# SiftScience/kafka-assigner

Measured on NVIDIA H100. Metric: partition-replica assignments/sec, higher is better.
Workload: dtype int32

## Files before the change

### kafka_assigner_b200/csrc/kassign.cu

```cuda
#include "kassign_stage.cuh"
#include "kassign_order.cuh"
#include "kassign_json.cuh"
#include "kassign_score.cuh"
#include "kassign_waves.cuh"
#include "kassign_waves_json.cuh"

#include <algorithm>
#include <climits>
#include <cmath>
#include <cstdio>
#include <cstdlib>
#include <cstring>
#include <map>
#include <new>
#include <string>
#include <unordered_map>
#include <vector>

#include "../../include/kassign.h"

namespace {

constexpr int KA_SM_COUNT_FALLBACK = 132;
constexpr size_t KA_SMEM_BUDGET = 200 * 1024;
// ... 162 lines not shown

template <typename F>
void for_each_event(ka_ctx* c, F f) {
    const struct { cudaEvent_t* e; size_t n; bool timed; } pools[] = {
        {c->ev, sizeof(c->ev) / sizeof(cudaEvent_t), true},
        {&c->ev_pipe[0][0], sizeof(c->ev_pipe) / sizeof(cudaEvent_t), true},
        {&c->ev_chain[0][0], sizeof(c->ev_chain) / sizeof(cudaEvent_t), true},
        {&c->ev_in, 1, false},
        {c->ev_stage, KA_MAX_BLOCKS, false},
        {&c->ev_chain_in, 1, false},
        {c->ev_b1, KA_MAX_CHAIN_EVENTS, false},
        {c->ev_b2, KA_MAX_CHAIN_EVENTS, false},
        {&c->ev_emit_done, 1, false},
        {c->ev_json_in, KA_MAX_JSON_FRAGS, false},
        {c->ev_json_scan, KA_MAX_JSON_FRAGS, false},
        {&c->ev_out_done, 1, false},
    };
    for (const auto& p : pools)
        for (size_t i = 0; i < p.n; ++i) f(p.e[i], p.timed);
}

int park_counters(ka_ctx* c) {
    if (c->br.N == 0 || !c->d_ctr8.p) return KA_OK;
    std::vector<int32_t> h((size_t)c->br.N * KA_MAX_SLOTS);
    KA_CUDA(cudaMemcpy(h.data(), c->d_ctr8.p, h.size() * 4, cudaMemcpyDeviceToHost));
    for (int i = 0; i < c->br.N; ++i) {
        const int32_t* row = h.data() + (size_t)i * KA_MAX_SLOTS;
        bool nz = false;
        for (int r = 0; r < KA_MAX_SLOTS; ++r) nz |= row[r] != 0;
        if (nz) c->parked[c->broker_id[i]] = std::vector<int32_t>(row, row + KA_MAX_SLOTS);
        else c->parked.erase(c->broker_id[i]);
    }
    return KA_OK;
}

int check_brokers(int N, const int32_t* broker_id, const int32_t* broker_rack) {
    if (N < 0 || (N > 0 && (!broker_id || !broker_rack))) return KA_ERR_BAD_ARG;
    if (N > 65535) return KA_ERR_LIMIT;
    for (int i = 0; i < N; ++i) {
        if (i > 0 && broker_id[i] <= broker_id[i - 1]) return KA_ERR_BAD_ARG;
        if (broker_rack[i] < 0 || broker_rack[i] >= 65535) return KA_ERR_BAD_ARG;
    }
    return KA_OK;
}

struct BrokerTable {
    int lut_mode = KA_LUT_SMEM, min_id = 0, lut_off = 0;
    uint32_t range = 0;
    std::vector<uint16_t> blob, glut;
    int blob_bytes() const { return (int)(blob.size() * 2); }
    KaBrokers device(int N, const uint16_t* d_blob, const uint16_t* d_glut, const int32_t* d_broker_id) const {
        return KaBrokers{N, lut_mode, lut_off, blob_bytes(), min_id, range, d_blob, d_glut, d_broker_id};
    }
};

BrokerTable broker_table(int N, const int32_t* broker_id, const int32_t* broker_rack) {
    BrokerTable t;
    t.min_id = N > 0 ? broker_id[0] : 0;
    const uint64_t range64 = N > 0 ? (uint64_t)((int64_t)broker_id[N - 1] - (int64_t)broker_id[0]) + 1 : 0;
    const size_t npad = align16((size_t)std::max(N, 1) * 2) / 2;
    std::vector<uint16_t> rackc(std::max(N, 1), 0);
    {
        std::unordered_map<int32_t, int> seen;
        for (int i = 0; i < N; ++i) {
            auto it = seen.find(broker_rack[i]);
            if (it == seen.end()) it = seen.emplace(broker_rack[i], (int)seen.size()).first;
            rackc[i] = (uint16_t)it->second;
        }
    }
    size_t lut_elems = 0;
    if (range64 <= KA_LUT_SMEM_MAX_RANGE) {
        t.lut_mode = KA_LUT_SMEM;
        t.range = (uint32_t)range64;
        lut_elems = align16((size_t)std::max<uint64_t>(range64, 1) * 2) / 2;
    } else if (range64 <= KA_LUT_GLOBAL_MAX_RANGE) {
        t.lut_mode = KA_LUT_GLOBAL;
        t.range = (uint32_t)range64;
        t.glut.assign((size_t)range64, (uint16_t)KA_DEAD);
        for (int i = 0; i < N; ++i) t.glut[(size_t)((int64_t)broker_id[i] - t.min_id)] = (uint16_t)i;
    } else {
        t.lut_mode = KA_LUT_BSEARCH;
        t.range = 0;
    }
    t.lut_off = (int)npad;
    t.blob.assign(npad + lut_elems, (uint16_t)KA_DEAD);
    for (int i = 0; i < N; ++i) {
        t.blob[i] = rackc[i];
        if (t.lut_mode == KA_LUT_SMEM) t.blob[npad + (size_t)((int64_t)broker_id[i] - t.min_id)] = (uint16_t)i;
    }
    return t;
}

constexpr size_t KA_ORDER_SMEM_BUDGET = 226 * 1024;

int make_plan(int N, int blob_bytes, int64_t Q, int S, int Pmax, int64_t capmax, bool ragged, Plan& pl, ka_status* st) {
    if (Q >= (int64_t)1 << 31) return set_status(st, KA_ERR_LIMIT, -1, -1, INT_MAX, 0);
    pl.a_blob_bytes = blob_bytes;
    pl.a_load_kind = capmax <= 255 ? 0 : 1;
    const int lsz = pl.a_load_kind == 0 ? 1 : 2;
    pl.a_load_bytes = (int)align16((size_t)std::max(N, 1) * lsz);
    pl.a_slab_bytes = (int)align16((size_t)std::max(Pmax, 1) * S * 2);
    pl.a_cnt_bytes = (int)align16((size_t)std::max(Pmax, 1));
    pl.a_levels = (capmax > 1 || ragged) ? 1 : 0;
    if (pl.a_levels && Pmax > 32767) return set_status(st, KA_ERR_LIMIT, -1, -1, Pmax, N);
    pl.lv_owner_bytes = pl.a_levels ? (int)align16((size_t)std::max(N, 1) * 4) : 0;
    pl.lv_last_bytes = pl.a_levels ? (int)align16((size_t)std::max(N, 1) * 2) : 0;
    pl.lv_p_bytes = pl.a_levels ? (int)align16((size_t)(std::max(Pmax, 1) + 2) * 2) : 0;
    const size_t per_warp = (size_t)pl.a_load_bytes + pl.a_slab_bytes + pl.a_cnt_bytes + pl.lv_owner_bytes + pl.lv_last_bytes +
                            2 * (size_t)pl.lv_p_bytes;
    const size_t shared = 16 + (size_t)blob_bytes;
    if (shared + per_warp > KA_SMEM_BUDGET) return set_status(st, KA_ERR_LIMIT, -1, -1, Pmax, N);
    pl.a_warps = (int)std::min<size_t>(16, (KA_SMEM_BUDGET - shared) / per_warp);
    pl.a_smem = shared + per_warp * pl.a_warps;
    pl.rec_kind = S <= 3 ? 3 : (S == 4 ? 4 : 8);
    pl.rec_bytes = pl.rec_kind == 3 ? 16 : 32;
    const int cw = pl.rec_kind == 8 ? 8 : 4;
    const int max_nt = pl.rec_kind == 3 ? 1024 : (pl.rec_kind == 4 ? 512 : 256);
    const size_t ctr_bytes = pl.rec_kind == 3 ? (size_t)(std::max(N, 1) + 1) * 4 : (size_t)std::max(N, 1) * cw * 4;
    const int lg_max = pl.rec_kind == 3 ? 10 : 9, lg_min = 7;
    auto ring_bytes = [&](int l) { return ((size_t)KA_RING_STAGES << l) * pl.rec_bytes + 256; };
    int lg = lg_max;
    pl.b_gctr = 0;
    while (lg > lg_min && ctr_bytes + ring_bytes(lg) > KA_ORDER_SMEM_BUDGET) --lg;
    if (ctr_bytes + ring_bytes(lg) > KA_ORDER_SMEM_BUDGET) {
        pl.b_gctr = 1;
        lg = lg_max;
    }
    if (const char* e = std::getenv("KA_ORDER_GLOBAL_CTR")) pl.b_gctr = pl.b_gctr || std::atoi(e);
    pl.b_ring_log2 = lg;
    pl.b_smem = ring_bytes(lg) + (pl.b_gctr ? 0 : ctr_bytes);
    int64_t width = pl.a_levels ? std::min<int64_t>(Pmax, std::max<int64_t>(1, N / std::max(S, 1) / 2)) : Pmax;
    const int64_t cuts = (std::max<int64_t>(width, 1) + max_nt - 1) / max_nt;
    width = (std::max<int64_t>(width, 1) + cuts - 1) / cuts;
    int nt = (int)std::min<int64_t>(max_nt, ((width + 31) / 32) * 32);
    if (const char* e = std::getenv("KA_ORDER_THREADS")) nt = std::atoi(e);
    nt = std::max(32, std::min(max_nt, (nt / 32) * 32));
    nt = std::min(nt, (KA_RING_STAGES - 1) << lg);
    pl.b_threads = nt;
    return KA_OK;
}

template <typename K>
cudaError_t allow_smem(K kernel, size_t bytes) {
    return cudaFuncSetAttribute(kernel, cudaFuncAttributeMaxDynamicSharedMemorySize, (int)bytes);
}

struct Shape {
    int T = 0, P = 0, RF = 0, desired_rf = -1, S = 1;
    const int32_t* d_hash = nullptr;
    const int32_t* d_cur = nullptr;
    const int64_t* d_part_off = nullptr;
    const int64_t* d_rep_off = nullptr;
    int64_t Q = 0, R = 0;
    int Pmax = 0;
    int64_t capmax = 0;
};

int64_t dense_capmax(int P, int rf_t, int n) {
    return n > 0 && rf_t <= n ? ((int64_t)P * std::max(rf_t, 0) + n - 1) / n : 0;
}

Shape dense_shape(int T, int P, int RF, int desired_rf, int S, int N, const int32_t* d_hash = nullptr, const int32_t* d_cur = nullptr) {
    Shape sh{T, P, RF, desired_rf, S, d_hash, d_cur};
    sh.Q = (int64_t)T * P;
    sh.R = sh.Q * RF;
    sh.Pmax = P;
    sh.capmax = dense_capmax(P, desired_rf >= 0 ? desired_rf : RF, N);
    return sh;
}

Shape ragged_shape(int T, int64_t Q, int64_t R, int desired_rf, int S, int Pmax = 0, int64_t capmax = 0) {
    Shape sh{T, 0, 0, desired_rf, S};
    sh.Q = Q;
    sh.R = R;
    sh.Pmax = Pmax;
    sh.capmax = capmax;
    return sh;
}

int describe_block(const Shape& sh, int t0, int t1, int blk, int N, int blob_bytes, StageDesc& d, ka_status* st) {
    const bool ragged = sh.d_part_off != nullptr;
    d = StageDesc();
    d.topic_base = t0;
    d.T = t1 - t0;
    d.blk = blk;
    d.q0 = (int64_t)t0 * sh.P;
    d.Q = ragged ? sh.Q : (int64_t)d.T * sh.P;
    d.d_hash = sh.d_hash + t0;
    d.d_part_off = sh.d_part_off;
    d.d_rep_off = sh.d_rep_off;
    d.P = sh.P;
    d.RF = sh.RF;
    d.d_cur = sh.d_cur + d.q0 * sh.RF;
    d.desired_rf = sh.desired_rf;
    d.S = sh.S;
    d.Pmax = sh.Pmax;
    d.capmax = sh.capmax;
    return make_plan(N, blob_bytes, d.Q, d.S, d.Pmax, d.capmax, ragged, d.pl, st);
}

int reserve_scratch(ka_ctx* c, const StageDesc* ds, int K) {
    const StageDesc& e = ds[K - 1];
    const size_t q = (size_t)std::max<int64_t>(e.q0 + e.Q, 1);
    const size_t T = (size_t)std::max(e.topic_base + e.T, 1);
    KA_CUDA(c->run.reserve(q * ds[0].pl.rec_bytes + 256, q, T, T + K + 1, ds[0].pl.a_levels, 16));
    return KA_OK;
}

int reserve_io(ka_ctx* c, Shape& sh, bool ragged) {
    KA_CUDA(c->d_hash.reserve((size_t)std::max(sh.T, 1) * 4));
    if (ragged) {
        KA_CUDA(c->d_part_off.reserve((size_t)(sh.T + 1) * 8));
        KA_CUDA(c->d_rep_off.reserve((size_t)(sh.Q + 1) * 8));
    }
    KA_CUDA(c->d_cur.reserve((size_t)std::max<int64_t>(sh.R, 1) * 4));
    KA_CUDA(c->d_out.reserve((size_t)std::max<int64_t>(sh.Q, 1) * sh.S * 4));
    KA_CUDA(c->d_out_len.reserve((size_t)std::max<int64_t>(sh.Q, 1) * 4));
    sh.d_hash = c->d_hash.as<int32_t>();
    sh.d_cur = c->d_cur.as<int32_t>();
    if (ragged) {
        sh.d_part_off = c->d_part_off.as<int64_t>();
        sh.d_rep_off = c->d_rep_off.as<int64_t>();
    }
    return KA_OK;
}

int reset_flags(ka_ctx* c, cudaStream_t s) {
    c->h_pin->err_topic = -1;
    c->h_pin->spin_flag = -1;
    c->chain_used = 0;
    c->slot_timed[0] = c->slot_timed[1] = false;
    KA_CUDA(cudaMemsetAsync(c->run.flags.p, 0xFF, 2 * sizeof(int), s));
    return KA_OK;
}

template <typename LoadT, bool LEVELS, int SM, bool CAND>
cudaError_t launch_stage_t(ka_ctx* c, cudaStream_t s, const KaSolveParams& p, const Plan& pl, int T, int ncand, int* grid_x) {
    auto kern = ka_sticky_spread_kernel<LoadT, LEVELS, SM, CAND>;
    const int threads = pl.a_warps * 32;
    cudaError_t e = allow_smem(kern, pl.a_smem);
    if (e != cudaSuccess) return e;
    int occ = 1;
    e = cudaOccupancyMaxActiveBlocksPerMultiprocessor(&occ, kern, threads, pl.a_smem);
    if (e != cudaSuccess) return e;
    int grid = (T + pl.a_warps - 1) / pl.a_warps;
    grid = std::min(grid, std::max(1, std::max(1, occ) * c->sm_count / std::max(ncand, 1)));
    *grid_x = grid;
    kern<<<dim3(grid, std::max(ncand, 1)), threads, pl.a_smem, s>>>(p, pl.a_load_bytes, pl.a_slab_bytes, pl.a_cnt_bytes, pl.lv_owner_bytes,
                                                                 pl.lv_last_bytes, pl.lv_p_bytes);
    return cudaGetLastError();
}

template <typename LoadT, bool LEVELS, bool CAND>
cudaError_t launch_stage(ka_ctx* c, cudaStream_t s, const KaSolveParams& p, const Plan& pl, int T, int ncand, int* grid_x) {
    return p.S <= 3 ? launch_stage_t<LoadT, LEVELS, 3, CAND>(c, s, p, pl, T, ncand, grid_x)
                    : launch_stage_t<LoadT, LEVELS, 8, CAND>(c, s, p, pl, T, ncand, grid_x);
}

void reset_plans(ka_ctx* c) {
    for (int32_t& v : c->order_plan) v = 0;
    for (int32_t& v : c->stage_plan) v = 0;
}

template <bool CAND>
int launch_stage_plan(ka_ctx* c, cudaStream_t s, const KaSolveParams& p, const Plan& pl, int T, int ncand, int lut_mask) {
    cudaError_t e;
    int grid_x = 0;
    if (!pl.a_levels) e = launch_stage<uint8_t, false, CAND>(c, s, p, pl, T, ncand, &grid_x);
    else if (pl.a_load_kind == 0) e = launch_stage<uint8_t, true, CAND>(c, s, p, pl, T, ncand, &grid_x);
    else e = launch_stage<uint16_t, true, CAND>(c, s, p, pl, T, ncand, &grid_x);
    KA_CUDA(e);
    c->launches++;
    int32_t* r = c->stage_plan;
    r[0] = pl.a_load_kind == 0 ? 1 : 2;
    r[1] = pl.a_levels;
    r[2] = p.S <= 3 ? 3 : 8;
    r[3] = ncand;
    r[4] = pl.a_warps;
    r[5] = grid_x;
    r[6] = lut_mask;
    r[7]++;
    return KA_OK;
}

KaSolveParams stage_params(const StageDesc& d) {
    KaSolveParams p{};
    p.T = d.T;
    p.topic_base = d.topic_base;
    p.topic_hash = d.d_hash;
    p.part_off = d.d_part_off;
    p.P = d.P;
    p.rep_off = d.d_rep_off;
    p.RF = d.RF;
    p.cur = d.d_cur;
    p.desired_rf = d.desired_rf;
    p.S = d.S;
    p.Pmax = d.Pmax;
    p.blob_space = d.pl.a_blob_bytes;
    p.rec_kind = d.pl.rec_kind;
    p.chunk_w = d.pl.b_threads;
    return p;
}

int enq_stage(ka_ctx* c, cudaStream_t s, const StageDesc& d, cudaEvent_t a_done) {
    const Plan& pl = d.pl;
    RunScratch& r = c->run;
    if (d.T > 0) {
        KaSolveParams p = stage_params(d);
        p.br = c->br;
        p.out.rec = r.rec.as<unsigned char>() + (size_t)d.q0 * pl.rec_bytes;
        p.out.perm = pl.a_levels ? r.perm.as<uint16_t>() + d.q0 : nullptr;
        p.out.ntl = pl.a_levels ? r.ntl.as<int32_t>() + d.topic_base : nullptr;
        p.out.lend = pl.a_levels ? r.lend.as<uint32_t>() + d.q0 : nullptr;
        p.out.tstatus = r.tstatus.as<int4>();
        p.out.err_topic = r.flags.as<unsigned>();
        const int rc = launch_stage_plan<false>(c, s, p, pl, d.T, 0, 1 << c->br.lut_mode);
        if (rc != KA_OK) return rc;
    }
    if (c->timing) KA_CUDA(cudaEventRecord(a_done, s));
    if (pl.a_levels && d.T > 0) {
        int32_t* ntl = r.ntl.as<int32_t>() + d.topic_base;
        int32_t* loff = r.loff.as<int32_t>() + d.topic_base + d.blk;
        ka_level_scan_kernel<<<1, 1024, 0, s>>>(ntl, d.T, loff);
        KA_CUDA(cudaGetLastError());
        ka_level_fill_kernel<<<(d.T + 7) / 8, 256, 0, s>>>(ntl, loff, r.lend.as<uint32_t>() + d.q0, d.d_part_off, d.P, d.T, d.T, d.Q,
                                                            r.lvl_end.as<uint32_t>() + d.q0);
        KA_CUDA(cudaGetLastError());
        c->launches += 2;
    }
    return KA_OK;
}

template <int KIND, int MAXNT, bool CAND, bool GCTR, bool SINGLE, bool WARP1, bool FULL>
cudaError_t launch_order_t(cudaStream_t s, const KaOrderParams& o, const Plan& pl, int ncand, bool behind) {
    auto kern = ka_order_levels_kernel<KIND, GCTR, MAXNT, SINGLE, WARP1, FULL, CAND>;
    cudaError_t e = allow_smem(kern, pl.b_smem);
    if (e != cudaSuccess) return e;
    cudaLaunchAttribute attr{};
    attr.id = cudaLaunchAttributeProgrammaticStreamSerialization;
    attr.val.programmaticStreamSerializationAllowed = 1;
    cudaLaunchConfig_t cfg{};
    cfg.gridDim = dim3(CAND ? ncand : 1);
    cfg.blockDim = dim3(pl.b_threads);
    cfg.dynamicSmemBytes = pl.b_smem;
    cfg.stream = s;
    cfg.attrs = &attr;
    cfg.numAttrs = behind ? 1 : 0;
    return cudaLaunchKernelEx(&cfg, kern, o);
}

template <int KIND, int MAXNT, bool CAND = false>
cudaError_t launch_order(cudaStream_t s, const KaOrderParams& o, const Plan& pl, int* sel, int ncand = 0, bool behind = false) {
    if constexpr (KIND > 1) {
        *sel = pl.b_gctr ? 4 : 0;
        return pl.b_gctr ? launch_order_t<KIND, MAXNT, false, true, false, false, false>(s, o, pl, ncand, behind)
                         : launch_order_t<KIND, MAXNT, false, false, false, false, false>(s, o, pl, ncand, behind);
    } else {
        const bool warp1 = pl.b_threads == 32;
        const bool single = !warp1 && o.uniform_width != 0 && o.uniform_width <= (uint32_t)pl.b_threads;
        const bool full = single && o.uniform_width == (uint32_t)pl.b_threads;
        *sel = (pl.b_gctr ? 4 : 0) | (warp1 ? 1 : (full ? 3 : (single ? 2 : 0)));
        switch (*sel) {
            case 0: return launch_order_t<KIND, MAXNT, CAND, false, false, false, false>(s, o, pl, ncand, behind);
            case 1: return launch_order_t<KIND, MAXNT, CAND, false, false, true, false>(s, o, pl, ncand, behind);
            case 2: return launch_order_t<KIND, MAXNT, CAND, false, true, false, false>(s, o, pl, ncand, behind);
            case 3: return launch_order_t<KIND, MAXNT, CAND, false, true, false, true>(s, o, pl, ncand, behind);
            case 4: return launch_order_t<KIND, MAXNT, CAND, true, false, false, false>(s, o, pl, ncand, behind);
            case 5: return launch_order_t<KIND, MAXNT, CAND, true, false, true, false>(s, o, pl, ncand, behind);
            case 6: return launch_order_t<KIND, MAXNT, CAND, true, true, false, false>(s, o, pl, ncand, behind);
            default: return launch_order_t<KIND, MAXNT, CAND, true, true, false, true>(s, o, pl, ncand, behind);
        }
    }
}

void note_order(ka_ctx* c, const Plan& pl, int sel, int ncand) {
    int32_t* r = c->order_plan;
    r[0] = pl.rec_kind;
    r[1] = pl.a_levels;
    r[2] = pl.b_threads;
    r[3] = pl.b_ring_log2;
    r[4] = (sel >> 2) & 1;
    r[5] = sel & 3;
    r[6]++;
    r[7] = ncand;
}

constexpr int KA_CHAIN_SUB_TOPICS = 512;
constexpr int KA_CHAIN_LARGE_BLOCK = 1024;

int chain_subblocks(const StageDesc& d, int blocks_in_solve, bool overlapped = false) {
    if (d.d_part_off || d.pl.rec_kind != 3 || d.T < 2) return 1;
    int n = std::max(1, 8 / std::max(1, blocks_in_solve));
    n = std::min(n, std::max(1, d.T / 128));
    if (overlapped && d.T >= KA_CHAIN_LARGE_BLOCK) n = std::max(n, d.T / KA_CHAIN_SUB_TOPICS);
    if (const char* e = std::getenv("KA_CHAIN_SUBBLOCKS")) n = std::max(1, std::min(std::atoi(e), d.T));
    return std::min(n, KA_MAX_CHAIN_BLOCKS);
}

struct SolveCall {
    const int32_t* h_hash = nullptr;
    const int32_t* h_cur = nullptr;
    const int64_t* h_part_off = nullptr;
    const int64_t* h_rep_off = nullptr;
    const int32_t* h_part_id = nullptr;
    int32_t* d_part_id = nullptr;
    int32_t* d_out = nullptr;
    int32_t* d_out_len = nullptr;
    int32_t* h_out = nullptr;
    int32_t* h_out_len = nullptr;
    bool json = false;
    bool stream_out = false;
    int json_blocks = 0;
    int chains = 0;
    bool emits = false;

    SolveCall(int32_t* out, int32_t* out_len) : d_out(out), d_out_len(out_len) {}
};

SolveCall host_call(ka_ctx* c, const int32_t* topic_hash, const int64_t* part_off, const int64_t* rep_off, const int32_t* cur_broker,
                    int32_t* out_len, int32_t* out_broker, const int32_t* part_id = nullptr) {
    SolveCall io(c->d_out.as<int32_t>(), c->d_out_len.as<int32_t>());
    io.h_hash = topic_hash;
    io.h_part_off = part_off;
    io.h_rep_off = rep_off;
    io.h_cur = cur_broker;
    io.h_part_id = part_id;
    io.d_part_id = part_id ? c->d_part_id.as<int32_t>() : nullptr;
    io.h_out = out_broker;
    io.h_out_len = out_len;
    return io;
}

struct SubBlock { int t0, t1; int64_t r0, rq; };

SubBlock sub_block(const StageDesc& d, int j, int nsub) {
    SubBlock b;
    b.t0 = (int)((int64_t)d.T * j / nsub);
    b.t1 = (int)((int64_t)d.T * (j + 1) / nsub);
    b.r0 = d.d_part_off ? 0 : (int64_t)b.t0 * d.P;
    b.rq = d.d_part_off ? d.Q : (int64_t)(b.t1 - b.t0) * d.P;
    return b;
}

KaJsonParams json_params(ka_ctx* c, const int32_t* out, const int32_t* out_len, int S, int T, const int64_t* part_off,
                         const int32_t* part_id, int64_t row0, int64_t rows, unsigned long long cap) {
    KaJsonParams p{};
    p.Q = (uint32_t)rows;
    p.row0 = (uint32_t)row0;
    p.T = T;
    p.part_off = part_off;
    p.part_id = part_id;
    p.name_off = c->d_name_off.as<int64_t>();
    p.names = c->d_names.as<char>();
    p.out = out + row0 * S;
    p.out_len = out_len + row0;
    p.S = S;
    p.rowlen = c->d_json_rowlen.as<uint32_t>() + row0;
    p.json = c->d_json.as<char>();
    p.cap = cap;
    return p;
}

KaJsonParams json_fragment(ka_ctx* c, const StageDesc& d, const SolveCall& io, int64_t row0, int64_t rows, int k) {
    KaJsonParams p = json_params(c, io.d_out, io.d_out_len, d.S, d.T, d.d_part_off, io.d_part_id, row0, rows,
                                 (unsigned long long)c->d_json.cap);
    p.blocksum = c->d_json_blocksum.as<uint32_t>() + (row0 / 256) + k;
    p.total = c->d_json_state.as<unsigned long long>();
    p.frag = p.total + 2 + 2 * k;
    return p;
}

template <bool SEG>
void enq_json_lengths(cudaStream_t s, const KaJsonParams& p, const KaJsonSegs& sg) {
    const int nblocks = (int)((p.Q + 255) / 256);
    if (nblocks > 0) ka_json_len_kernel<SEG><<<nblocks, 256, 0, s>>>(p, sg);
    ka_json_scan_kernel<<<1, 1024, 0, s>>>(p, nblocks);
}

template <typename K, typename... A>
cudaError_t enq_json_write(K kernel, unsigned grid, cudaStream_t s, const A&... args) {
    const cudaError_t e = allow_smem(kernel, KA_JSON_SMEM_BYTES + 16);
    if (e == cudaSuccess) kernel<<<grid, 256, KA_JSON_SMEM_BYTES + 16, s>>>(args...);
    return e;
}

int enq_json_rows(ka_ctx* c, cudaStream_t s_done, SolveCall& io, const StageDesc& d, const SubBlock& b, bool first, bool last) {
    const int k = io.json_blocks;
    if (k >= KA_MAX_JSON_FRAGS) return KA_ERR_LIMIT;
    KA_CUDA(cudaEventRecord(c->ev_json_in[k], s_done));
    KA_CUDA(cudaStreamWaitEvent(c->sj, c->ev_json_in[k], 0));
    KaJsonParams p = json_fragment(c, d, io, d.q0 + b.r0, b.rq, k);
    p.P = std::max(d.P, 1);
    p.topic0 = d.topic_base + b.t0;
    p.first = first;
    p.last = last;
    enq_json_lengths<false>(c->sj, p, KaJsonSegs{});
    KA_CUDA(enq_json_write(ka_json_write_kernel<false>, std::max((p.Q + 255) / 256, 1u), c->sj, p, KaJsonSegs{}));
    KA_CUDA(cudaGetLastError());
    KA_CUDA(cudaMemcpyAsync(c->h_frag + 2 * k, p.frag, 16, cudaMemcpyDeviceToHost, c->sj));
    KA_CUDA(cudaEventRecord(c->ev_json_scan[k], c->sj));
    c->launches += 3;
    io.json_blocks = k + 1;
    return KA_OK;
}

int64_t json_fragment_rows(int64_t Q) {
    const int64_t spread = (Q + KA_MAX_JSON_FRAGS - 1) / KA_MAX_JSON_FRAGS;
    return std::max(KA_JSON_FRAG_ROWS, (spread + 255) / 256 * 256);
}

int enq_json(ka_ctx* c, cudaStream_t s_done, SolveCall& io, const StageDesc& d, const SubBlock& b, bool first, bool last) {
    if (!d.d_part_off) return enq_json_rows(c, s_done, io, d, b, first, last);
    const int64_t step = json_fragment_rows(b.rq);
    int64_t r = 0;
    do {
        SubBlock f = b;
        f.r0 = b.r0 + r;
        f.rq = std::min(step, b.rq - r);
        const int rc = enq_json_rows(c, s_done, io, d, f, first && r == 0, last && r + step >= b.rq);
        if (rc != KA_OK) return rc;
        r += step;
    } while (r < b.rq);
    return KA_OK;
}

int enq_copy_out(cudaStream_t s, const SolveCall& io, int S, int64_t r0, int64_t rows) {
    KA_CUDA(cudaMemcpyAsync(io.h_out + r0 * S, io.d_out + r0 * S, (size_t)rows * S * 4, cudaMemcpyDeviceToHost, s));
    if (io.h_out_len) KA_CUDA(cudaMemcpyAsync(io.h_out_len + r0, io.d_out_len + r0, (size_t)rows * 4, cudaMemcpyDeviceToHost, s));
    return KA_OK;
}

KaOrderParams order_params(ka_ctx* c, const StageDesc& d, const SubBlock& b) {
    const Plan& pl = d.pl;
    KaOrderParams o{};
    o.N = c->br.N;
    o.S = d.S;
    o.uniform_width = pl.a_levels ? 0u : (uint32_t)d.P;
    o.chunk_end = pl.a_levels ? c->run.lvl_end.as<uint32_t>() + d.q0 : nullptr;
    o.ctr8 = c->d_ctr8.as<int32_t>();
    o.ring_log2 = pl.b_ring_log2;
    const int32_t* loff = pl.a_levels ? c->run.loff.as<int32_t>() + d.topic_base + d.blk : nullptr;
    o.Q = (uint32_t)b.rq;
    o.rec = c->run.rec.as<unsigned char>() + (size_t)(d.q0 + b.r0) * pl.rec_bytes;
    o.pos_base = (uint32_t)b.r0;
    o.chunk_lo_ptr = loff ? loff + b.t0 : nullptr;
    o.chunk_hi_ptr = loff ? loff + b.t1 : nullptr;
    return o;
}

int enq_slot_chain(ka_ctx* c, cudaStream_t s, const StageDesc& d, int slot, int j, int nsub, bool behind = false) {
    const SubBlock b = sub_block(d, j, nsub);
    if (b.rq <= 0 || c->br.N <= 0) return KA_OK;
    const KaOrderParams o = order_params(c, d, b);
    int sel = 0;
    KA_CUDA((slot == 0 ? launch_order<0, 1024>(s, o, d.pl, &sel, 0, behind) : launch_order<1, 1024>(s, o, d.pl, &sel, 0, behind)));
    note_order(c, d.pl, sel, 0);
    c->launches++;
    return KA_OK;
}

int enq_emit_block(ka_ctx* c, cudaStream_t s, const StageDesc& d, int j, int nsub, int32_t* d_out, int32_t* d_out_len) {
    const Plan& pl = d.pl;
    const SubBlock b = sub_block(d, j, nsub);
    if (b.rq <= 0 || c->br.N <= 0) return KA_OK;
    ka_emit3_kernel<<<(unsigned)((b.rq + 255) / 256), 256, 0, s>>>(
        reinterpret_cast<const uint4*>(c->run.rec.as<unsigned char>() + (size_t)(d.q0 + b.r0) * pl.rec_bytes),
        pl.a_levels ? c->run.perm.as<uint16_t>() + d.q0 + b.r0 : nullptr, d.d_part_off, b.t1 - b.t0, d.P, c->d_broker_id.as<int32_t>(),
        (uint32_t)b.rq, d.S, d_out + (size_t)b.r0 * d.S, d_out_len ? d_out_len + b.r0 : nullptr, c->d_ctr8.as<int32_t>());
    KA_CUDA(cudaGetLastError());
    c->launches++;
    return KA_OK;
}

int enq_order_emit(ka_ctx* c, cudaStream_t s, const StageDesc& d, SolveCall& io, int blocks_in_solve) {
    const int S = d.S;
    const Plan& pl = d.pl;
    if (d.Q <= 0 || c->br.N <= 0) return io.json && d.d_part_off && d.Q == 0 ? enq_json(c, s, io, d, sub_block(d, 0, 1), true, true) : KA_OK;
    int32_t* d_out = io.d_out + d.q0 * S;
    int32_t* d_out_len = io.d_out_len ? io.d_out_len + d.q0 : nullptr;
    if (pl.rec_kind != 3) {
        const SubBlock b = sub_block(d, 0, 1);
        KaOrderParams o = order_params(c, d, b);
        o.broker_id = c->d_broker_id.as<int32_t>();
        o.out = d_out;
        o.out_len = d_out_len;
        int sel = 0;
        KA_CUDA((pl.rec_kind == 4 ? launch_order<4, 512>(s, o, pl, &sel) : launch_order<8, 256>(s, o, pl, &sel)));
        note_order(c, pl, sel, 0);
        c->launches++;
        if (io.json) return enq_json(c, s, io, d, b, d.blk == 0, d.blk == blocks_in_solve - 1);
        return KA_OK;
    }
    const int nsub = chain_subblocks(d, blocks_in_solve, true);
    const int e = c->chain_used;
    if (e >= KA_MAX_BLOCKS || io.chains + nsub > KA_MAX_CHAIN_EVENTS) return KA_ERR_LIMIT;
    cudaStream_t s1 = c->sb1, se = c->sj;
    if (c->timing) KA_CUDA(cudaEventRecord(c->ev_chain[e][0], s1));
    for (int j = 0; j < nsub; ++j) {
        const int k = io.chains + j;
        int rc = enq_slot_chain(c, s1, d, 0, j, nsub, true);
        if (rc != KA_OK) return rc;
        KA_CUDA(cudaEventRecord(c->ev_b1[k], s1));
        KA_CUDA(cudaStreamWaitEvent(s, c->ev_b1[k], 0));
        if (c->timing && j == 0) KA_CUDA(cudaEventRecord(c->ev_chain[e][2], s));
        if ((rc = enq_slot_chain(c, s, d, 1, j, nsub, true)) != KA_OK) return rc;
        KA_CUDA(cudaEventRecord(c->ev_b2[k], s));
        KA_CUDA(cudaStreamWaitEvent(se, c->ev_b2[k], 0));
        if ((rc = enq_emit_block(c, se, d, j, nsub, d_out, d_out_len)) != KA_OK) return rc;
        if (j == nsub - 1) {
            if (c->timing) KA_CUDA(cudaEventRecord(c->ev_chain[e][3], se));
            KA_CUDA(cudaEventRecord(c->ev_emit_done, se));
            io.emits = true;
        }
        const SubBlock b = sub_block(d, j, nsub);
        if (io.stream_out && (rc = enq_copy_out(se, io, S, d.q0 + b.r0, b.rq)) != KA_OK) return rc;
        if (io.json && (rc = enq_json(c, se, io, d, b, d.blk == 0 && j == 0, d.blk == blocks_in_solve - 1 && j == nsub - 1)) != KA_OK)
            return rc;
    }
    if (c->timing) KA_CUDA(cudaEventRecord(c->ev_chain[e][1], s1));
    io.chains += nsub;
    c->chain_used = e + 1;
    return KA_OK;
}

int join_emits(ka_ctx* c, cudaStream_t s, const SolveCall& io) {
    if (io.emits) KA_CUDA(cudaStreamWaitEvent(s, c->ev_emit_done, 0));
    return KA_OK;
}

int chain_fork(ka_ctx* c, cudaStream_t s) {
    KA_CUDA(cudaEventRecord(c->ev_chain_in, s));
    KA_CUDA(cudaStreamWaitEvent(c->sb1, c->ev_chain_in, 0));
    return KA_OK;
}

int enq_solve_end(ka_ctx* c, cudaStream_t s) {
    KA_CUDA(cudaMemcpyAsync(&c->h_pin->err_topic, c->run.flags.p, 2 * sizeof(int), cudaMemcpyDeviceToHost, s));
    if (c->timing) {
        KA_CUDA(cudaEventRecord(c->ev[5], s));
        c->ev_valid = true;
    }
    return KA_OK;
}

int pipeline_stages(int T, int64_t Q) {
    int k = Q >= 262144 ? std::min(4, T / 2048) : 1;
    if (const char* e = std::getenv("KA_PIPELINE_STAGES")) k = std::atoi(e);
    return std::max(1, std::min(k, std::min(KA_MAX_BLOCKS, std::max(T, 1))));
}

int enq_inputs(cudaStream_t s, const SolveCall& io, const StageDesc& d, int64_t ncur) {
    auto h2d = [&](const void* dst, const void* src, size_t bytes) {
        return cudaMemcpyAsync(const_cast<void*>(dst), src, bytes, cudaMemcpyHostToDevice, s);
    };
    if (io.h_hash && d.T > 0) KA_CUDA(h2d(d.d_hash, io.h_hash + d.topic_base, (size_t)d.T * 4));
    if (io.h_part_off && d.T > 0) KA_CUDA(h2d(d.d_part_off, io.h_part_off, (size_t)(d.T + 1) * 8));
    if (io.h_rep_off && d.Q > 0) KA_CUDA(h2d(d.d_rep_off, io.h_rep_off, (size_t)(d.Q + 1) * 8));
    if (io.h_part_id && d.Q > 0) KA_CUDA(h2d(io.d_part_id, io.h_part_id, (size_t)d.Q * 4));
    if (io.h_cur && ncur > 0) KA_CUDA(h2d(d.d_cur, io.h_cur + d.q0 * d.RF, (size_t)ncur * 4));
    return KA_OK;
}

int run_solve(ka_ctx* c, cudaStream_t s, const Shape& sh, SolveCall& io, ka_status* st) {
    c->staged = false;
    c->last_was_staged = false;
    reset_plans(c);
    const bool ragged = sh.d_part_off != nullptr;
    const int T = sh.T;
    const int K = ragged ? 1 : pipeline_stages(T, (int64_t)T * sh.P);
    const bool host_io = (io.h_cur != nullptr || io.h_out != nullptr) && K >= 3;
    const int wsum = host_io ? 2 * (K - 1) : K;
    auto bound = [&](int k) { return k <= 0 ? 0 : (k >= K ? T : (int)((int64_t)T * (host_io ? 2 * k - 1 : k) / wsum)); };
    StageDesc ds[KA_MAX_BLOCKS];
    int rc;
    for (int k = 0; k < K; ++k)
        if ((rc = describe_block(sh, bound(k), bound(k + 1), k, c->br.N, c->br.blob_bytes, ds[k], st)) != KA_OK) return rc;
    if ((rc = reserve_scratch(c, ds, K)) != KA_OK) return rc;
    c->last_stages = K;
    if (c->timing) KA_CUDA(cudaEventRecord(c->ev[0], s));
    if (K == 1) {
        const StageDesc& d = ds[0];
        if ((rc = enq_inputs(s, io, d, ragged ? sh.R : d.Q * d.RF)) != KA_OK) return rc;
        if ((rc = reset_flags(c, s)) != KA_OK) return rc;
        if (c->timing) KA_CUDA(cudaEventRecord(c->ev[1], s));
        if ((rc = enq_stage(c, s, d, c->ev[2])) != KA_OK) return rc;
        if (c->timing) KA_CUDA(cudaEventRecord(c->ev[3], s));
        if ((rc = chain_fork(c, s)) != KA_OK) return rc;
        if ((rc = enq_order_emit(c, s, d, io, 1)) != KA_OK || (rc = join_emits(c, s, io)) != KA_OK) return rc;
        if (c->timing) KA_CUDA(cudaEventRecord(c->ev[4], s));
        if (io.h_out && d.Q > 0 && c->br.N > 0 && (rc = enq_copy_out(s, io, d.S, 0, d.Q)) != KA_OK) return rc;
    } else {
        cudaStream_t aux = c->aux;
        io.stream_out = io.h_out && ds[0].pl.rec_kind == 3 && !io.json;
        KA_CUDA(cudaEventRecord(c->ev_in, s));
        if (io.stream_out) KA_CUDA(cudaStreamWaitEvent(c->sj, c->ev_in, 0));
        KA_CUDA(cudaStreamWaitEvent(aux, c->ev_in, 0));
        if ((rc = reset_flags(c, aux)) != KA_OK) return rc;
        for (int k = 0; k < K; ++k) {
            const StageDesc& d = ds[k];
            if ((rc = enq_inputs(aux, io, d, d.Q * d.RF)) != KA_OK) return rc;
            if (c->timing) KA_CUDA(cudaEventRecord(c->ev_pipe[k][0], aux));
            if ((rc = enq_stage(c, aux, d, c->ev_pipe[k][1])) != KA_OK) return rc;
            if (c->timing) KA_CUDA(cudaEventRecord(c->ev_pipe[k][2], aux));
            KA_CUDA(cudaEventRecord(c->ev_stage[k], aux));
        }
        for (int k = 0; k < K; ++k) {
            const StageDesc& d = ds[k];
            KA_CUDA(cudaStreamWaitEvent(s, c->ev_stage[k], 0));
            KA_CUDA(cudaStreamWaitEvent(c->sb1, c->ev_stage[k], 0));
            if (k == 0) KA_CUDA(cudaStreamWaitEvent(c->sb1, c->ev_in, 0));
            if (c->timing) KA_CUDA(cudaEventRecord(c->ev_pipe[k][3], s));
            if ((rc = enq_order_emit(c, s, d, io, K)) != KA_OK) return rc;
            if (c->timing) KA_CUDA(cudaEventRecord(c->ev_pipe[k][4], s));
            if (io.h_out && !io.stream_out && d.Q > 0 && c->br.N > 0 && (rc = enq_copy_out(s, io, d.S, d.q0, d.Q)) != KA_OK) return rc;
        }
        if ((rc = join_emits(c, s, io)) != KA_OK) return rc;
        if (io.stream_out) {
            KA_CUDA(cudaEventRecord(c->ev_out_done, c->sj));
            KA_CUDA(cudaStreamWaitEvent(s, c->ev_out_done, 0));
        }
    }
    return enq_solve_end(c, s);
}

ka_status topic_status(int t, const int4& ts, const int32_t* part_id, const int64_t* part_off) {
    ka_status r;
    set_status(&r, ts.x, t, ts.y >= 0 && part_id && part_off ? part_id[part_off[t] + ts.y] : ts.y, ts.z, ts.w);
    return r;
}

int finish_status(ka_ctx* c, cudaStream_t s, ka_status* st, const int32_t* part_id = nullptr, const int64_t* part_off = nullptr) {
    KA_CUDA(cudaStreamSynchronize(s));
    c->pending_status = false;
    ka_status r{};
    set_status(&r, KA_OK);
    if (c->h_pin->err_topic != -1) {
        const int t = c->h_pin->err_topic;
        KA_CUDA(cudaMemcpy(&c->h_pin->tstatus, c->run.tstatus.as<int4>() + t, sizeof(int4), cudaMemcpyDeviceToHost));
        r = topic_status(t, c->h_pin->tstatus, part_id, part_off);
        r.topic_index += c->last_was_staged ? c->topic_base : 0;
    }
    if (c->timing && c->ev_valid) {
        for (int i = 0; i < 8; ++i) c->last_ms[i] = 0.f;
        cudaEventElapsedTime(&c->last_ms[5], c->ev[0], c->ev[5]);
        if (c->last_stages <= 1) {
            cudaEventElapsedTime(&c->last_ms[3], c->ev[0], c->ev[1]);
            cudaEventElapsedTime(&c->last_ms[0], c->ev[1], c->ev[2]);
            cudaEventElapsedTime(&c->last_ms[1], c->ev[2], c->ev[3]);
            cudaEventElapsedTime(&c->last_ms[7], c->ev[3], c->ev[4]);
            cudaEventElapsedTime(&c->last_ms[4], c->ev[4], c->ev[5]);
        } else {
            for (int k = 0; k < c->last_stages; ++k) {
                float a = 0.f, t = 0.f, b = 0.f;
                cudaEventElapsedTime(&a, c->ev_pipe[k][0], c->ev_pipe[k][1]);
                cudaEventElapsedTime(&t, c->ev_pipe[k][1], c->ev_pipe[k][2]);
                cudaEventElapsedTime(&b, c->ev_pipe[k][3], c->ev_pipe[k][4]);
                c->last_ms[0] += a;
                c->last_ms[1] += t;
                c->last_ms[7] += b;
            }
        }
        if (c->chain_used > 0) {
            for (int e = 0; e < c->chain_used; ++e) {
                float b1 = 0.f, b2 = 0.f;
                cudaEventElapsedTime(&b1, c->ev_chain[e][0], c->ev_chain[e][1]);
                cudaEventElapsedTime(&b2, c->ev_chain[e][2], c->ev_chain[e][3]);
                c->last_ms[2] += b1;
                c->last_ms[6] += b2;
            }
        } else if (c->slot_timed[0] || c->slot_timed[1]) {
            if (c->slot_timed[0]) cudaEventElapsedTime(&c->last_ms[2], c->ev_chain[0][0], c->ev_chain[0][1]);
            if (c->slot_timed[1]) cudaEventElapsedTime(&c->last_ms[6], c->ev_chain[1][0], c->ev_chain[1][1]);
        } else {
            c->last_ms[2] = c->last_ms[7];
        }
    }
    c->last = r;
    if (st) *st = r;
    return r.code;
}

int enter(ka_ctx* c, bool collect) {
    KA_CUDA(cudaSetDevice(c->device));
    if (collect && c->pending_status) finish_status(c, c->last_stream, nullptr);
    return KA_OK;
}

int finish(ka_ctx* c, cudaStream_t s, ka_status* st, bool sync, const int32_t* part_id = nullptr, const int64_t* part_off = nullptr) {
    c->last_stream = s;
    c->pending_status = true;
    return st || sync ? finish_status(c, s, st, part_id, part_off) : KA_OK;
}

int fail_members(ka_status* st, int K, int rc) {
    for (int k = 0; k < K; ++k) set_status(st + k, rc);
    return rc;
}

int abort_batch(ka_ctx* c, cudaStream_t s, ka_status* st, int K, int rc) {
    cudaStreamSynchronize(c->sb1);
    cudaStreamSynchronize(s);
    return fail_members(st, K, rc);
}

int batch_args(ka_ctx* c, int K, int out_stride, ka_status* st) {
    if (!st || K < 0) return KA_ERR_BAD_ARG;
    for (int k = 0; k < K; ++k) set_status(st + k, KA_OK);
    if (!c) return fail_members(st, K, KA_ERR_NO_DEVICE);
    if (K > KA_MAX_CANDIDATES || out_stride > 3) return fail_members(st, K, KA_ERR_LIMIT);
    if (out_stride < 1) return fail_members(st, K, KA_ERR_BAD_ARG);
    return KA_OK;
}

int check_tables(int K, const int32_t* cand_off, const int32_t* broker_id, const int32_t* broker_rack) {
    if (!cand_off || cand_off[0] != 0) return KA_ERR_BAD_ARG;
    for (int k = 0; k < K; ++k) {
        const int n = cand_off[k + 1] - cand_off[k];
        if (cand_off[k + 1] < cand_off[k] || (n > 0 && (!broker_id || !broker_rack))) return KA_ERR_BAD_ARG;
        const int rc = n > 0 ? check_brokers(n, broker_id + cand_off[k], broker_rack + cand_off[k]) : KA_OK;
        if (rc != KA_OK) return rc;
    }
    return KA_OK;
}

struct BatchMember {
    int tab = 0;
    int t0 = 0, T = 0;
    int64_t row0 = 0, Q = 0;
    int desired_rf = -1;
    int64_t rec0 = 0;
    int64_t topic0 = 0;
    int n = 0, blob_bytes = 0;
    int Pmax = 0;
    int64_t capmax = 0;
    int S = 1;
};

struct Batch {
    int K = 0;
    const int32_t* cand_off = nullptr;
    const int32_t* broker_id = nullptr;
    std::vector<BrokerTable> tabs;
    std::vector<BatchMember> m;
    int64_t recs = 0;
    int topics = 0;
    int fill_T = 0;
    int64_t fill_rows = 0;
    int64_t out_rows = 0;
    int nmax = 0, blob_max = 0, Pmax = 0, Tmax = 0;
    int64_t capmax = 0, Qmax = 0;

    void add(const BatchMember& mb) {
        m.push_back(mb);
        nmax = std::max(nmax, mb.n);
        blob_max = std::max(blob_max, mb.blob_bytes);
        Pmax = std::max(Pmax, mb.Pmax);
        capmax = std::max(capmax, mb.capmax);
        Tmax = std::max(Tmax, mb.T);
        Qmax = std::max(Qmax, mb.Q);
    }
};

int batch_tables(ka_ctx* c, int K, const int32_t* cand_off, const int32_t* broker_id, const int32_t* broker_rack, int64_t recs,
                 Batch& b, ka_status* st) {
    if (recs >= ((int64_t)1 << 31)) return fail_members(st, K, KA_ERR_LIMIT);
    const int rc = enter(c, true);
    if (rc != KA_OK) return fail_members(st, K, rc);
    reset_plans(c);
    b.K = K;
    b.cand_off = cand_off;
    b.broker_id = broker_id;
    b.tabs.resize(K);
    for (int k = 0; k < K; ++k)
        b.tabs[k] = broker_table(cand_off[k + 1] - cand_off[k], broker_id + cand_off[k], broker_rack + cand_off[k]);
    return KA_OK;
}

void add_candidates(Batch& b, int T, int64_t Q, int Pmax, int desired_rf, const std::vector<int64_t>& capmax) {
    const int64_t q = std::max<int64_t>(Q, 1);
    for (int k = 0; k < b.K; ++k)
        b.add(BatchMember{k, 0, T, 0, Q, desired_rf, (int64_t)k * q, (int64_t)k * T, b.cand_off[k + 1] - b.cand_off[k],
                          b.tabs[k].blob_bytes(), Pmax, capmax[k]});
    b.recs = (int64_t)b.K * q;
    b.topics = b.K * T;
    b.fill_T = T;
    b.fill_rows = Q;
    b.out_rows = Q;
}

void add_clusters(Batch& b, int T, int64_t Q, const std::vector<BatchMember>& passed, ka_status* st) {
    for (BatchMember mb : passed) {
        mb.blob_bytes = b.tabs[mb.tab].blob_bytes();
        Plan own;
        if (make_plan(mb.n, mb.blob_bytes, mb.Q, mb.S, mb.Pmax, mb.capmax, true, own, st + mb.tab) == KA_OK) b.add(mb);
    }
    b.recs = std::max<int64_t>(Q, 1);
    b.topics = T;
    b.fill_T = std::max(T, 1);
    b.out_rows = 0;
    if (b.Tmax == 0) b.m.clear();
}

int plan_batch(Shape sh, const Batch& b, StageDesc& d, ka_status* st) {
    sh.Pmax = b.Pmax;
    sh.capmax = b.capmax;
    const int rc = describe_block(sh, 0, sh.T, 0, b.nmax, b.blob_max, d, st);
    for (int k = 1; k < b.K && rc != KA_OK; ++k) st[k] = st[0];
    return rc;
}

int finish_batch(ka_ctx* c, cudaStream_t s, const Batch& b, ka_status* st, const int32_t* part_id = nullptr,
                 const int64_t* part_off = nullptr) {
    const int K = b.K, M = (int)b.m.size();
    if (cudaStreamSynchronize(s) != cudaSuccess) return fail_members(st, K, KA_ERR_CUDA);
    std::vector<unsigned> err(std::max(M, 1));
    if (M > 0 && cudaMemcpy(err.data(), c->batch_run.flags.p, (size_t)M * 4, cudaMemcpyDeviceToHost) != cudaSuccess)
        return fail_members(st, K, KA_ERR_CUDA);
    for (int k = 0; k < M; ++k) {
        if (err[k] == 0xFFFFFFFFu) continue;
        const BatchMember& mb = b.m[k];
        const int t = (int)err[k] - mb.t0;
        int4 ts;
        if (cudaMemcpy(&ts, c->batch_run.tstatus.as<int4>() + mb.topic0 + t, sizeof(int4), cudaMemcpyDeviceToHost) != cudaSuccess)
            return fail_members(st, K, KA_ERR_CUDA);
        st[mb.tab] = topic_status(mb.t0 + t, ts, part_id, part_off);
        st[mb.tab].topic_index = t;
    }
    for (int k = 0; k < K; ++k)
        if (st[k].code != KA_OK) return st[k].code;
    return KA_OK;
}

template <typename F>
void enq_wave_peaks(ka_ctx* c, cudaStream_t s, const KaWaveBucket* log, unsigned n, int N, typename F::S* sum) {
    const unsigned blocks = (unsigned)std::max<int64_t>(1, std::min<int64_t>(((int64_t)n + 255) / 256, (int64_t)c->sm_count * 8));
    ka_wave_peak_kernel<false, F><<<blocks, 256, 0, s>>>(log, n, N, sum);
    ka_wave_peak_kernel<true, F><<<blocks, 256, 0, s>>>(log, n, N, sum);
    c->launches += 2;
}

}

extern "C" {

const char* ka_version(void) { return "kassign-b200 0.1 (sm_90a)"; }

int32_t ka_java_string_hash(const char* s) {
    uint32_t h = 0;
    const unsigned char* u = reinterpret_cast<const unsigned char*>(s);
    while (*u) {
        uint32_t cp;
        int extra;
        unsigned char b = *u++;
        if (b < 0x80) { cp = b; extra = 0; }
        else if ((b & 0xE0) == 0xC0) { cp = b & 0x1F; extra = 1; }
        else if ((b & 0xF0) == 0xE0) { cp = b & 0x0F; extra = 2; }
        else if ((b & 0xF8) == 0xF0) { cp = b & 0x07; extra = 3; }
        else { cp = 0xFFFD; extra = 0; }
        while (extra-- > 0 && *u) cp = (cp << 6) | (*u++ & 0x3F);
        if (cp >= 0x10000) {
            cp -= 0x10000;
            h = h * 31u + (0xD800u + (cp >> 10));
            h = h * 31u + (0xDC00u + (cp & 0x3FFu));
        } else {
            h = h * 31u + cp;
        }
    }
    return (int32_t)h;
}

int32_t ka_rack_indices(int32_t N, const int32_t* broker_id, const char* const* rack_name, int32_t* broker_rack) {
    if (N < 0 || (N > 0 && (!broker_id || !broker_rack))) return KA_ERR_BAD_ARG;
    std::map<std::string, int32_t> key2idx;
    for (int i = 0; i < N; ++i) {
        std::string key = (rack_name && rack_name[i]) ? std::string(rack_name[i]) : std::to_string(broker_id[i]);
        auto it = key2idx.find(key);
        if (it == key2idx.end()) it = key2idx.emplace(key, (int32_t)key2idx.size()).first;
        broker_rack[i] = it->second;
    }
    return KA_OK;
}

ka_ctx* ka_ctx_create(int32_t device) {
    int ndev = 0;
    if (cudaGetDeviceCount(&ndev) != cudaSuccess || ndev <= 0 || device < 0 || device >= ndev) {
        cudaGetLastError();
        return nullptr;
    }
    if (cudaSetDevice(device) != cudaSuccess) return nullptr;
    ka_ctx* c = new (std::nothrow) ka_ctx();
    if (!c) return nullptr;
    c->device = device;
    cudaDeviceProp prop;
    if (cudaGetDeviceProperties(&prop, device) == cudaSuccess) c->sm_count = prop.multiProcessorCount;
    bool ok = cudaHostAlloc(reinterpret_cast<void**>(&c->h_pin), sizeof(HostPinned), cudaHostAllocDefault) == cudaSuccess &&
              cudaHostAlloc(reinterpret_cast<void**>(&c->h_frag), 2 * KA_MAX_JSON_FRAGS * sizeof(unsigned long long),
                            cudaHostAllocDefault) == cudaSuccess;
    for (cudaStream_t* s : {&c->stream, &c->aux, &c->sb1, &c->sj})
        ok = ok && cudaStreamCreateWithFlags(s, cudaStreamNonBlocking) == cudaSuccess;
    for_each_event(c, [&](cudaEvent_t& e, bool timed) {
        ok = ok && cudaEventCreateWithFlags(&e, timed ? cudaEventDefault : cudaEventDisableTiming) == cudaSuccess;
    });
    if (!ok) {
        ka_ctx_destroy(c);
        return nullptr;
    }
    return c;
}

void ka_ctx_destroy(ka_ctx* c) {
    if (!c) return;
    cudaSetDevice(c->device);
    for (cudaStream_t s : {c->stream, c->aux, c->sb1, c->sj})
        if (s) cudaStreamSynchronize(s);
    for (DevBuf* b : {&c->d_blob, &c->d_glut, &c->d_broker_id, &c->d_ctr8, &c->d_hash, &c->d_part_off, &c->d_rep_off, &c->d_cur,
                      &c->d_out, &c->d_out_len, &c->d_json, &c->d_names, &c->d_name_off, &c->d_part_id, &c->d_json_rowlen,
                      &c->d_json_blocksum, &c->d_json_state, &c->d_batch_tab, &c->d_batch_ctr, &c->d_score_w, &c->d_score_sum,
                      &c->d_score_brk, &c->d_score_off, &c->d_json_seg, &c->d_wv_nrecv, &c->d_wv_wave, &c->d_wv_tmp, &c->d_wv_rec,
                      &c->d_wv_cnt, &c->d_wv_state, &c->d_wv_log, &c->d_wv_sum, &c->d_wv_meta, &c->d_wv_perm, &c->d_wv_hist, &c->d_wv_doc,
                      &c->d_wv_part, &c->d_wv_jump, &c->d_wv_send, &c->d_wv_slog, &c->d_wv_ssum})
        b->release();
    c->run.release();
    c->batch_run.release();
    for_each_event(c, [](cudaEvent_t& e, bool) {
        if (e) cudaEventDestroy(e);
    });
    for (cudaStream_t s : {c->stream, c->aux, c->sb1, c->sj})
        if (s) cudaStreamDestroy(s);
    if (c->h_pin) cudaFreeHost(c->h_pin);
    if (c->h_frag) cudaFreeHost(c->h_frag);
    delete c;
}

int32_t ka_ctx_reset(ka_ctx* c) {
    if (!c) return KA_ERR_NO_DEVICE;
    int rc = enter(c, true);
    if (rc != KA_OK) return rc;
    c->parked.clear();
    if (c->br.N > 0 && c->d_ctr8.p) KA_CUDA(cudaMemset(c->d_ctr8.p, 0, (size_t)c->br.N * KA_MAX_SLOTS * 4));
    return KA_OK;
}

int32_t ka_ctx_set_brokers(ka_ctx* c, int32_t N, const int32_t* broker_id, const int32_t* broker_rack) {
    if (!c) return KA_ERR_NO_DEVICE;
    int rc = check_brokers(N, broker_id, broker_rack);
    if (rc != KA_OK) return rc;
    if ((rc = enter(c, true)) != KA_OK || (rc = park_counters(c)) != KA_OK) return rc;

    const BrokerTable t = broker_table(N, broker_id, broker_rack);
    if (t.lut_mode == KA_LUT_GLOBAL) {
        KA_CUDA(c->d_glut.reserve(t.glut.size() * 2));
        KA_CUDA(cudaMemcpy(c->d_glut.p, t.glut.data(), t.glut.size() * 2, cudaMemcpyHostToDevice));
    }
    KA_CUDA(c->d_blob.reserve(t.blob.size() * 2));
    KA_CUDA(cudaMemcpy(c->d_blob.p, t.blob.data(), t.blob.size() * 2, cudaMemcpyHostToDevice));
    KA_CUDA(c->d_broker_id.reserve((size_t)std::max(N, 1) * 4));
    if (N > 0) KA_CUDA(cudaMemcpy(c->d_broker_id.p, broker_id, (size_t)N * 4, cudaMemcpyHostToDevice));
    c->br = t.device(N, c->d_blob.as<uint16_t>(), c->d_glut.as<uint16_t>(), c->d_broker_id.as<int32_t>());
    c->broker_id.assign(broker_id, broker_id + N);
    std::vector<int32_t> h((size_t)(std::max(N, 1) + 1) * KA_MAX_SLOTS, 0);
    for (int i = 0; i < N; ++i) {
        auto it = c->parked.find(broker_id[i]);
        if (it != c->parked.end()) std::copy(it->second.begin(), it->second.end(), h.begin() + (size_t)i * KA_MAX_SLOTS);
    }
    KA_CUDA(c->d_ctr8.reserve(h.size() * 4));
    KA_CUDA(cudaMemcpy(c->d_ctr8.p, h.data(), h.size() * 4, cudaMemcpyHostToDevice));
    return KA_OK;
}

int32_t ka_ctx_counter_slots(ka_ctx*) { return KA_MAX_SLOTS; }

int32_t ka_ctx_get_counters(ka_ctx* c, int32_t* counter) {
// ... 1387 lines not shown
```

Baseline: 3.143 billion.

## Defer side-stream stage waits into the slot chain and record stage events earlier

The secondary chain stream no longer waits for each stage's completion event at the top of the per-stage loop. Instead, the wait for the next stage is inserted just before that stage's last sub-block, or after the order step for non-chain record kinds. The stage-done event is now recorded inside the stage enqueue, before the level-table kernels whenever those tables are not needed. The aim is to let order and slot-chain work for one stage overlap with the staging of the next, trading per-stage timing detail for fewer serialization points. Timing now records one span across all stages instead of per-stage spans.

```diff
diff --git a/kafka_assigner_b200/csrc/kassign.cu b/kafka_assigner_b200/csrc/kassign.cu
--- a/kafka_assigner_b200/csrc/kassign.cu
+++ b/kafka_assigner_b200/csrc/kassign.cu
@@ -488,7 +488,7 @@
     return p;
 }
 
-int enq_stage(ka_ctx* c, cudaStream_t s, const StageDesc& d, cudaEvent_t a_done) {
+int enq_stage(ka_ctx* c, cudaStream_t s, const StageDesc& d, cudaEvent_t a_done, cudaEvent_t done = nullptr) {
     const Plan& pl = d.pl;
     RunScratch& r = c->run;
     if (d.T > 0) {
@@ -503,8 +503,10 @@
         const int rc = launch_stage_plan<false>(c, s, p, pl, d.T, 0, 1 << c->br.lut_mode);
         if (rc != KA_OK) return rc;
     }
+    const bool tables = pl.a_levels && d.T > 0;
+    if (done && !tables) KA_CUDA(cudaEventRecord(done, s));
     if (c->timing) KA_CUDA(cudaEventRecord(a_done, s));
-    if (pl.a_levels && d.T > 0) {
+    if (tables) {
         int32_t* ntl = r.ntl.as<int32_t>() + d.topic_base;
         int32_t* loff = r.loff.as<int32_t>() + d.topic_base + d.blk;
         ka_level_scan_kernel<<<1, 1024, 0, s>>>(ntl, d.T, loff);
@@ -513,6 +515,7 @@
                                                             r.lvl_end.as<uint32_t>() + d.q0);
         KA_CUDA(cudaGetLastError());
         c->launches += 2;
+        if (done) KA_CUDA(cudaEventRecord(done, s));
     }
     return KA_OK;
 }
@@ -758,9 +761,10 @@
     return KA_OK;
 }
 
-int enq_order_emit(ka_ctx* c, cudaStream_t s, const StageDesc& d, SolveCall& io, int blocks_in_solve) {
+int enq_order_emit(ka_ctx* c, cudaStream_t s, const StageDesc& d, SolveCall& io, int blocks_in_solve, cudaEvent_t next_stage = nullptr) {
     const int S = d.S;
     const Plan& pl = d.pl;
+    if (next_stage && (d.Q <= 0 || c->br.N <= 0 || pl.rec_kind != 3)) KA_CUDA(cudaStreamWaitEvent(c->sb1, next_stage, 0));
     if (d.Q <= 0 || c->br.N <= 0) return io.json && d.d_part_off && d.Q == 0 ? enq_json(c, s, io, d, sub_block(d, 0, 1), true, true) : KA_OK;
     int32_t* d_out = io.d_out + d.q0 * S;
     int32_t* d_out_len = io.d_out_len ? io.d_out_len + d.q0 : nullptr;
@@ -781,20 +785,22 @@
     const int e = c->chain_used;
     if (e >= KA_MAX_BLOCKS || io.chains + nsub > KA_MAX_CHAIN_EVENTS) return KA_ERR_LIMIT;
     cudaStream_t s1 = c->sb1, se = c->sj;
-    if (c->timing) KA_CUDA(cudaEventRecord(c->ev_chain[e][0], s1));
+    const int jw = nsub > 1 ? nsub - 1 : nsub;
+    if (c->timing && e == 0) KA_CUDA(cudaEventRecord(c->ev_chain[0][0], s1));
     for (int j = 0; j < nsub; ++j) {
         const int k = io.chains + j;
+        if (next_stage && j == jw) KA_CUDA(cudaStreamWaitEvent(s1, next_stage, 0));
         int rc = enq_slot_chain(c, s1, d, 0, j, nsub, true);
         if (rc != KA_OK) return rc;
         KA_CUDA(cudaEventRecord(c->ev_b1[k], s1));
         KA_CUDA(cudaStreamWaitEvent(s, c->ev_b1[k], 0));
-        if (c->timing && j == 0) KA_CUDA(cudaEventRecord(c->ev_chain[e][2], s));
+        if (c->timing && j == 0 && e == 0) KA_CUDA(cudaEventRecord(c->ev_chain[0][2], s));
         if ((rc = enq_slot_chain(c, s, d, 1, j, nsub, true)) != KA_OK) return rc;
         KA_CUDA(cudaEventRecord(c->ev_b2[k], s));
         KA_CUDA(cudaStreamWaitEvent(se, c->ev_b2[k], 0));
         if ((rc = enq_emit_block(c, se, d, j, nsub, d_out, d_out_len)) != KA_OK) return rc;
         if (j == nsub - 1) {
-            if (c->timing) KA_CUDA(cudaEventRecord(c->ev_chain[e][3], se));
+            if (c->timing) KA_CUDA(cudaEventRecord(c->ev_chain[0][3], se));
             KA_CUDA(cudaEventRecord(c->ev_emit_done, se));
             io.emits = true;
         }
@@ -803,7 +809,8 @@
         if (io.json && (rc = enq_json(c, se, io, d, b, d.blk == 0 && j == 0, d.blk == blocks_in_solve - 1 && j == nsub - 1)) != KA_OK)
             return rc;
     }
-    if (c->timing) KA_CUDA(cudaEventRecord(c->ev_chain[e][1], s1));
+    if (next_stage && jw == nsub) KA_CUDA(cudaStreamWaitEvent(s1, next_stage, 0));
+    if (c->timing && !next_stage) KA_CUDA(cudaEventRecord(c->ev_chain[0][1], s1));
     io.chains += nsub;
     c->chain_used = e + 1;
     return KA_OK;
@@ -886,18 +893,19 @@
             const StageDesc& d = ds[k];
             if ((rc = enq_inputs(aux, io, d, d.Q * d.RF)) != KA_OK) return rc;
             if (c->timing) KA_CUDA(cudaEventRecord(c->ev_pipe[k][0], aux));
-            if ((rc = enq_stage(c, aux, d, c->ev_pipe[k][1])) != KA_OK) return rc;
+            if ((rc = enq_stage(c, aux, d, c->ev_pipe[k][1], c->ev_stage[k])) != KA_OK) return rc;
             if (c->timing) KA_CUDA(cudaEventRecord(c->ev_pipe[k][2], aux));
-            KA_CUDA(cudaEventRecord(c->ev_stage[k], aux));
         }
         for (int k = 0; k < K; ++k) {
             const StageDesc& d = ds[k];
             KA_CUDA(cudaStreamWaitEvent(s, c->ev_stage[k], 0));
-            KA_CUDA(cudaStreamWaitEvent(c->sb1, c->ev_stage[k], 0));
-            if (k == 0) KA_CUDA(cudaStreamWaitEvent(c->sb1, c->ev_in, 0));
-            if (c->timing) KA_CUDA(cudaEventRecord(c->ev_pipe[k][3], s));
-            if ((rc = enq_order_emit(c, s, d, io, K)) != KA_OK) return rc;
-            if (c->timing) KA_CUDA(cudaEventRecord(c->ev_pipe[k][4], s));
+            if (k == 0) {
+                KA_CUDA(cudaStreamWaitEvent(c->sb1, c->ev_stage[0], 0));
+                KA_CUDA(cudaStreamWaitEvent(c->sb1, c->ev_in, 0));
+            }
+            if (c->timing && k == 0) KA_CUDA(cudaEventRecord(c->ev_pipe[0][3], s));
+            if ((rc = enq_order_emit(c, s, d, io, K, k + 1 < K ? c->ev_stage[k + 1] : nullptr)) != KA_OK) return rc;
+            if (c->timing && k == K - 1) KA_CUDA(cudaEventRecord(c->ev_pipe[K - 1][4], s));
             if (io.h_out && !io.stream_out && d.Q > 0 && c->br.N > 0 && (rc = enq_copy_out(s, io, d.S, d.q0, d.Q)) != KA_OK) return rc;
         }
         if ((rc = join_emits(c, s, io)) != KA_OK) return rc;
@@ -937,23 +945,17 @@
             cudaEventElapsedTime(&c->last_ms[4], c->ev[4], c->ev[5]);
         } else {
             for (int k = 0; k < c->last_stages; ++k) {
-                float a = 0.f, t = 0.f, b = 0.f;
+                float a = 0.f, t = 0.f;
                 cudaEventElapsedTime(&a, c->ev_pipe[k][0], c->ev_pipe[k][1]);
                 cudaEventElapsedTime(&t, c->ev_pipe[k][1], c->ev_pipe[k][2]);
-                cudaEventElapsedTime(&b, c->ev_pipe[k][3], c->ev_pipe[k][4]);
                 c->last_ms[0] += a;
                 c->last_ms[1] += t;
-                c->last_ms[7] += b;
             }
+            cudaEventElapsedTime(&c->last_ms[7], c->ev_pipe[0][3], c->ev_pipe[c->last_stages - 1][4]);
         }
         if (c->chain_used > 0) {
-            for (int e = 0; e < c->chain_used; ++e) {
-                float b1 = 0.f, b2 = 0.f;
-                cudaEventElapsedTime(&b1, c->ev_chain[e][0], c->ev_chain[e][1]);
-                cudaEventElapsedTime(&b2, c->ev_chain[e][2], c->ev_chain[e][3]);
-                c->last_ms[2] += b1;
-                c->last_ms[6] += b2;
-            }
+            cudaEventElapsedTime(&c->last_ms[2], c->ev_chain[0][0], c->ev_chain[0][1]);
+            cudaEventElapsedTime(&c->last_ms[6], c->ev_chain[0][2], c->ev_chain[0][3]);
         } else if (c->slot_timed[0] || c->slot_timed[1]) {
             if (c->slot_timed[0]) cudaEventElapsedTime(&c->last_ms[2], c->ev_chain[0][0], c->ev_chain[0][1]);
             if (c->slot_timed[1]) cudaEventElapsedTime(&c->last_ms[6], c->ev_chain[1][0], c->ev_chain[1][1]);
```

Result: faster. 3.263 billion (median of 6 runs) (+3.8%).
